# nullmax-vision/SimPB

Hardware: AMD Instinct MI355X
Metric: frames/sec (6-cam sample) + MSDeformAttn HBM GB/s, R50 704x256 @1/2/4/8 GPU (higher is better)
Workload: dtype f32

## Files before the change

### include/simpb_hip.h

```cpp
#ifndef SIMPB_HIP_H
#define SIMPB_HIP_H

#ifdef __cplusplus
extern "C" {
#endif

#define SIMPB_OK 0
#define SIMPB_EINVAL 1
#define SIMPB_ELAUNCH 2

#define SIMPB_RECORD3D_WIDTH 15

int simpb_abi_version(void);

const char* simpb_last_error(void);

#define SIMPB_KERNEL_DAF 1
#define SIMPB_KERNEL_MSDA 2
int simpb_timing_enable(int capacity);
int simpb_timing_read(int kernel_id, float* ms_out, int max_n);
void simpb_timing_reset(void);

int simpb_deformable_aggregation_forward(
    float* output, const float* mc_ms_feat, const int* spatial_shape, const int* scale_start_index,
// ... 77 lines not shown
                                       long long image_stride, int yoff, int iy, int irv, int igu, int igv, int ibu,
                                       void* stream);

int simpb_preprocess_mid_pitch(int out_width);

#define SIMPB_GEMM_MAX_SEGS 4
#define SIMPB_GEMM_MAX_JOBS 4
#define SIMPB_GEMM_OUT_F32 0
#define SIMPB_GEMM_OUT_SPLIT_HALFS 1
typedef struct simpb_gemm_job {
  const float* x[SIMPB_GEMM_MAX_SEGS];
  int ldx[SIMPB_GEMM_MAX_SEGS];
  int kseg[SIMPB_GEMM_MAX_SEGS];
  int num_seg;
  int M, N, K;
  const float* w;
  const float* bias;
  float* y;
  const int* m_live;
  int ldw, ldy, relu;
  int out_fmt;
  const int* row_flag;
  const float* bias2;
  const void* w_hi;
  const void* w_lo;
} simpb_gemm_job;
typedef struct simpb_gemm_args {
  int num_jobs;
  int reserved;
  simpb_gemm_job job[SIMPB_GEMM_MAX_JOBS];
} simpb_gemm_args;
int simpb_gemm_f32(const simpb_gemm_args* args, void* stream);

int simpb_layernorm_f32(float* out, int ldo, const float* x0, int ld0, int k0, const float* x1, int ld1, int k1,
                        const float* gamma, const float* beta, int num_rows, const int* m_live, void* stream);

#define SIMPB_MAX_LEVELS 8
int simpb_format_tokens(float* col_feats, const void* const* level_ptrs, const void* const* level_bias,
                        const int* level_hw, int num_levels, int num_images, int channels, int src_is_half, void* stream);

int simpb_bias_act_nhwc_f16(void* y, const void* bias, const void* residual, long long num_pixels, int channels,
                            int relu, void* stream);

int simpb_bias_relu_maxpool_nhwc_f16(void* y, const void* x, const void* bias, int num_images, int in_h, int in_w,
                                     int channels, void* stream);

int simpb_conv1x1_nhwc_f16(void* y, const void* x, const void* weight, const void* bias, const void* residual,
                           int num_images, int in_h, int in_w, int in_channels, int out_channels, int stride, int relu,
                           int residual_upsample2x, const void* input_bias, int variant, void* stream);

int simpb_conv3x3_nhwc_f16(void* y, float* tokens, void* tokens_f16, int tokens_per_cam, int level_start, const void* x,
                           const void* weight, const void* bias, int num_images, int in_h, int in_w, int in_channels,
                           int out_channels, int stride, int relu, int variant, void* stream);

int simpb_conv3x3_group_tokens_f16(int num_levels, float* tokens, void* tokens_f16, int tokens_per_cam, const int* level_start,
                                   const void* const* x, const void* const* weight, const void* const* bias, int num_images,
                                   const int* in_h, const int* in_w, int in_channels, int out_channels, int relu, void* stream);

int simpb_attention_f32(float* out, const float* q, const float* k, const float* v, const int* query_cam,
                        const int* group_start, int batch_size, int num_heads, int head_dim, int num_query,
                        int num_key, int ldq, int ldk, int ldv, int ldo, float scale, void* stream);

int simpb_attention_f32_split(float* out, const float* q, const float* k, const float* v, const int* query_cam,
                              const int* group_start, int batch_size, int num_heads, int head_dim, int num_query,
                              int num_key, int ldq, int ldk, int ldv, int ldo, float scale, void* stream);

int simpb_attention_split_halfs(float* out, const void* q, const void* k, const void* v, const int* query_cam,
                                const int* group_start, int batch_size, int num_heads, int head_dim, int num_query,
                                int num_key, int ldq, int ldk, int ldv, int ldo, void* stream);

#define SIMPB_MLP_MAX_OPS 12
#define SIMPB_MLP_MAX_CHAINS 8
#define SIMPB_MLP_POST_NONE 0
#define SIMPB_MLP_POST_REFINE3D 1
#define SIMPB_MLP_POST_REFINE2D 2
#define SIMPB_MLP_POST_SIGMOID 3
#define SIMPB_MLP_LINEAR 0
#define SIMPB_MLP_LAYERNORM 1
#define SIMPB_MLP_IN_ROWS 0
#define SIMPB_MLP_IN_SINE2D 1
#define SIMPB_MLP_IN_ROWS_LN 2
typedef struct simpb_mlp_op {
  int type, in_dim, out_dim, relu;
  const float* w;
  const float* b;
} simpb_mlp_op;
typedef struct simpb_mlp_chain {
  const float* x;
  const float* x2;
  float* out;
  const float* out_scale;
  int ldx, ldx2, ldo, in_dim, in_mode, n_ops;
  int post, ldres, res_cols, div_rows, div_col0, reserved;
  const float* res;
  const float* div;
  simpb_mlp_op ops[SIMPB_MLP_MAX_OPS];
  const float* ln_w;
  const float* ln_b;
  float* ln_out;
  int ld_ln_out, reserved2;
} simpb_mlp_chain;
typedef struct simpb_mlp_args {
  int num_rows, num_chains;
  int weights_transposed;
  int reserved;
  simpb_mlp_chain chain[SIMPB_MLP_MAX_CHAINS];
// ... 161 lines not shown
```

### simpb_amd/_lib.py

```python
import ctypes
import os

from .build import LIB

_lib = None

_P = ctypes.c_void_p
_I = ctypes.c_int
_F = ctypes.c_float
_LL = ctypes.c_longlong


class WorldTables(ctypes.Structure):
    _fields_ = [("class_range", _F * 32), ("attr_moving", ctypes.c_ubyte * 32), ("attr_still", ctypes.c_ubyte * 32),
                ("threshold", _F), ("has_threshold", _I), ("num_output", _I)]


SIGNATURES = {
    "simpb_abi_version": ([], _I),
    "simpb_last_error": ([], ctypes.c_char_p),
    "simpb_timing_enable": ([_I], _I),
    "simpb_timing_read": ([_I, _P, _I], _I),
    "simpb_timing_reset": ([], None),
    "simpb_deformable_aggregation_forward": ([_P] * 6 + [_I] * 8 + [_P], _I),
    "simpb_dfa_fused_forward": ([_P, _P, _I] + [_P] * 11 + [_I] * 9 + [_P], _I),
    "simpb_dfa_fused_forward_cams": ([_P, _P, _I] + [_P] * 11 + [_I] * 9 + [_P, _P], _I),
    "simpb_deformable_aggregation_backward": ([_P] * 9 + [_I] * 8 + [_P], _I),
    "simpb_ms_deform_attn_grouped_forward": ([_P] * 7 + [_I] * 8 + [_P], _I),
    "simpb_msda_linear_forward": ([_P, _I, _P, _I, _P, _P, _P, _I, _P, _I, _P, _P] + [_I] * 8 + [_P], _I),
    "simpb_ms_deform_attn_grouped_backward": ([_P] * 10 + [_I] * 8 + [_P], _I),
    "simpb_linear_f32": ([_P] * 4 + [_I] * 4 + [_P], _I),
    "simpb_linear_f16x3": ([_P] * 5 + [_I] * 3 + [_P], _I),
    "simpb_gemm_f32": ([_P, _P], _I),
    "simpb_layernorm_f32": ([_P, _I, _P, _I, _I, _P, _I, _I, _P, _P, _I, _P, _P], _I),
    "simpb_bias_act_nhwc_f16": ([_P, _P, _P, ctypes.c_longlong, _I, _I, _P], _I),
    "simpb_bias_relu_maxpool_nhwc_f16": ([_P, _P, _P, _I, _I, _I, _I, _P], _I),
    "simpb_conv1x1_nhwc_f16": ([_P] * 5 + [_I] * 8 + [_P, _I, _P], _I),
    "simpb_conv3x3_nhwc_f16": ([_P, _P, _P, _I, _I, _P, _P, _P] + [_I] * 8 + [_P], _I),
    "simpb_conv3x3_group_tokens_f16": ([_I, _P, _P, _I, _P, _P, _P, _P, _I, _P, _P, _I, _I, _I, _P], _I),
    "simpb_stem_conv7x7_pool_f16": ([_P] * 4 + [_I] * 4 + [_P], _I),
    "simpb_image_to_nhwc4_f16": ([_P, _P] + [ctypes.c_longlong] * 4 + [_I] * 4 + [_P], _I),
    "simpb_preprocess_u8_nhwc4_f16": ([_P] * 10 + [_I] * 11 + [_P], _I),
    "simpb_preprocess_yuv420sp_nhwc4_f16": ([_P] * 10 + [_I] * 18 + [_P], _I),
    "simpb_preprocess_surface_nhwc4_f16": ([_P] * 11 + [_I] * 12 + [_LL] * 4 + [_I] * 6 + [_P], _I),
    "simpb_preprocess_mid_pitch": ([_I], _I),
    "simpb_linear_f16in_split": ([_P] * 5 + [_I] * 3 + [_P], _I),
    "simpb_format_tokens": ([_P, _P, _P, _P, _I, _I, _I, _I, _P], _I),
    "simpb_attention_f32": ([_P] * 6 + [_I] * 9 + [_F, _P], _I),
    "simpb_attention_f32_split": ([_P] * 6 + [_I] * 9 + [_F, _P], _I),
    "simpb_attention_split_halfs": ([_P] * 6 + [_I] * 9 + [_P], _I),
    "simpb_mlp_chain_forward": ([_P, _P], _I),
    "simpb_bank_get": ([_P] * 6 + [_I] * 2 + [_F] * 2 + [_P], _I),
    "simpb_bank_update": ([_P] * 10 + [_I] * 5 + [_P], _I),
    "simpb_bank_update_rank": ([_P, _P] + [_I] * 4 + [_P], _I),
    "simpb_bank_update_merge": ([_P] * 13 + [_I, _P] + [_I] * 5 + [_P], _I),
    "simpb_bank_update_merge_active": ([_P] * 13 + [_I, _P] + [_I] * 5 + [_P, _P], _I),
    "simpb_bank_cache": ([_P] * 10 + [_I] * 6 + [_F, _I, _F, _P, _I, _P, _P], _I),
    "simpb_bank_cache_streams": ([_P] * 10 + [_I] * 6 + [_F, _I, _F, _P, _I, _P, _P, _P], _I),
    "simpb_bank_cache_streams_active": ([_P] * 10 + [_I] * 6 + [_F, _I, _F, _P, _I, _P, _P, _P, _P], _I),
    "simpb_decode3d_record": ([_P] * 6 + [_I] * 4 + [_P], _I),
    "simpb_decode2d_record": ([_P] * 6 + [_I] * 4 + [_F] * 4 + [_P], _I),
    "simpb_record2d_compact": ([_P, _LL, _P, _LL, _I, _I, _I, _P], _I),
    "simpb_decode2d_record_ragged": ([_P] * 7 + [_I] * 5 + [_F] * 4 + [_P], _I),
    "simpb_world_record": ([_P] * 5 + [WorldTables, _I, _P], _I),
    "simpb_topk_rows": ([_P, _P, _P, _I, _I, _I, _P], _I),
    "simpb_rowdot_sigmoid": ([_P, _P, _I, _P, _P, _I, _I, _P, _P], _I),
    "simpb_anchor_projection": ([_P] * 4 + [_I] * 2 + [_P], _I),
    "simpb_msda_prep": ([_P, _P, _P, _I, _P, _I, _P, _I, _I, _I, _I, _P, _P], _I),
    "simpb_dfa_points": ([_P] * 7 + [_I] * 5 + [_P], _I),
    "simpb_dfa_weights": ([_P] * 3 + [_I] * 6 + [_P], _I),
    "simpb_dfa_points_cams": ([_P] * 7 + [_I] * 5 + [_P, _P], _I),
    "simpb_dfa_weights_cams": ([_P] * 3 + [_I] * 6 + [_P, _P], _I),
    "simpb_alloc_project_cams": ([_P] * 5 + [_I] * 3 + [_F] * 5 + [_P, _P], _I),
    "simpb_alloc_project": ([_P] * 5 + [_I] * 3 + [_F] * 5 + [_P], _I),
    "simpb_alloc_compact": ([_P] * 3 + [_I] * 3 + [_P], _I),
    "simpb_alloc_group_start": ([_P] * 3 + [_I] * 3 + [_P], _I),
    "simpb_alloc_scatter": ([_P] * 12 + [_I] * 4 + [_F] * 2 + [_P], _I),
    "simpb_alloc_static": ([_P] * 15 + [_I] * 4 + [_F] * 5 + [_P], _I),
    "simpb_alloc_ragged": ([_P] * 15 + [_I] * 4 + [_F] * 5 + [_P], _I),
    "simpb_alloc_ragged_active": ([_P] * 15 + [_I] * 4 + [_F] * 5 + [_P, _P], _I),
    "simpb_alloc_static_cams": ([_P] * 15 + [_I] * 4 + [_F] * 5 + [_P, _P], _I),
    "simpb_alloc_ragged_cams": ([_P] * 15 + [_I] * 4 + [_F] * 5 + [_P, _P, _P], _I),
    "simpb_gather_rows": ([_P] * 3 + [_I] * 4 + [_P], _I),
    "simpb_aggregate_2d_to_3d": ([_P] * 8 + [_I] * 5 + [_P], _I),
    "simpb_aggregate_2d_to_3d_alpha": ([_P] * 9 + [_I, _I, _P, _P] + [_I] * 5 + [_P], _I),
}

ERRORS = {1: "SIMPB_EINVAL (bad pointer/size/layout)", 2: "SIMPB_ELAUNCH (kernel launch failed)"}


def lib():
# ... 23 lines not shown
```

### simpb_amd/csrc/conv1x1.hip

```cpp
#include <hip/hip_runtime.h>
#include <hip/hip_fp16.h>
#include <type_traits>
#include "../../include/simpb_hip.h"
#include "mfma_f16.h"

extern "C" int simpb_check_launch(void);
extern "C" int simpb_conv_pointwise_staged(void* y, const void* x, const void* weight, const void* bias, const void* residual,
                                           int p_out, int in_h, int in_w, int ho, int wo, int in_channels, int out_channels,
                                           int stride, int relu, int residual_upsample2x, int tiling, void* stream);

namespace {

using f32x16 = __attribute__((ext_vector_type(16))) float;
using h16x8 = __attribute__((ext_vector_type(8))) _Float16;

constexpr int BM = 128, BN = 64, BK = 64;
constexpr int LDH = BK + 8;
constexpr int LDC = BN + 1;
constexpr int kThreads = 256;

__device__ __forceinline__ int up2(int p, int Ho, int Wo) {
  const int n = p / (Ho * Wo), rem = p - n * (Ho * Wo);
  const int ho = rem / Wo, wo = rem - ho * Wo;
  return (n * (Ho >> 1) + (ho >> 1)) * (Wo >> 1) + (wo >> 1);
// ... 99 lines not shown
      __syncthreads();
      fetch(std::integral_constant<int, 1>{}, c + 3);
      multiply();
    }
  }

  __syncthreads();
#pragma unroll
  for (int n = 0; n < 2; ++n)
#pragma unroll
    for (int r = 0; r < 16; ++r) s_c[(wave * 32 + (r & 3) + 8 * (r >> 2) + 4 * kb) * LDC + n * 32 + r32] = acc[n][r];
  __syncthreads();
#pragma unroll
  for (int i = 0; i < 4; ++i) {
    const int idx = tid + i * kThreads;
    const int r = idx >> 3, c8 = (idx & 7) * 8;
    const int p = p0 + r;
    if (p >= P_out) continue;
    float v[8];
#pragma unroll
    for (int e = 0; e < 8; ++e) v[e] = s_c[r * LDC + c8 + e];
    if (full) {
      const h16x8 bv = *reinterpret_cast<const h16x8*>(bias + c0 + c8);
#pragma unroll
      for (int e = 0; e < 8; ++e) v[e] += (float)bv[e];
      if (residual) {
        const h16x8 rv = rres[i];
#pragma unroll
        for (int e = 0; e < 8; ++e) v[e] += (float)rv[e];
      }
      h16x8 o;
#pragma unroll
      for (int e = 0; e < 8; ++e) o[e] = (_Float16)(relu ? fmaxf(v[e], 0.f) : v[e]);
      *reinterpret_cast<h16x8*>(y + (size_t)p * Cout + c0 + c8) = o;
    } else {
#pragma unroll
      for (int e = 0; e < 8; ++e) {
        const int c = c0 + c8 + e;
        if (c < Cout) {
          float t = v[e] + (float)bias[c];
          if (residual) t += (float)residual[(size_t)(res_up ? up2(p, Ho, Wo) : p) * Cout + c];
          y[(size_t)p * Cout + c] = (_Float16)(relu ? fmaxf(t, 0.f) : t);
        }
      }
    }
  }
}

}

extern "C" int simpb_conv1x1_nhwc_f16(void* y, const void* x, const void* weight, const void* bias, const void* residual,
                                      int num_images, int in_h, int in_w, int in_channels, int out_channels, int stride,
                                      int relu, int residual_upsample2x, const void* input_bias, int variant, void* stream) {
  if (variant < 0 || variant > 3 || (input_bias && variant > 1)) return SIMPB_EINVAL;
  if (!y || !x || !weight || !bias || num_images <= 0 || in_h <= 0 || in_w <= 0 || in_channels <= 0 || out_channels <= 0 ||
      (stride != 1 && stride != 2) || in_channels % BK != 0 || out_channels % 8 != 0)
    return SIMPB_EINVAL;
  if ((reinterpret_cast<size_t>(y) | reinterpret_cast<size_t>(x) | reinterpret_cast<size_t>(weight) |
       reinterpret_cast<size_t>(bias) | reinterpret_cast<size_t>(residual) | reinterpret_cast<size_t>(input_bias)) & 15)
    return SIMPB_EINVAL;
  const int ho = (in_h - 1) / stride + 1, wo = (in_w - 1) / stride + 1;
  if (residual_upsample2x && (!residual || (ho & 1) || (wo & 1))) return SIMPB_EINVAL;
  const long long p_out = (long long)num_images * ho * wo;
  if (p_out > (1ll << 30)) return SIMPB_EINVAL;
  (void)hipGetLastError();
  if (variant == 0) {
    variant = (input_bias || in_channels < 512) ? 1 : 2;
  }
  if (variant > 1) {
    if ((long long)num_images * in_h * in_w * in_channels > (1ll << 31) - 1) return SIMPB_EINVAL;
    return simpb_conv_pointwise_staged(y, x, weight, bias, residual, (int)p_out, in_h, in_w, ho, wo, in_channels, out_channels,
                                       stride, relu, residual_upsample2x, variant - 2, stream);
  }
  dim3 grid((unsigned)((p_out + BM - 1) / BM), (out_channels + BN - 1) / BN);
  if (grid.y > 65535) return SIMPB_EINVAL;
  hipLaunchKernelGGL(conv1x1_f16_kernel, grid, dim3(kThreads), 0, static_cast<hipStream_t>(stream),
                     static_cast<_Float16*>(y), static_cast<const _Float16*>(x), static_cast<const _Float16*>(weight),
                     static_cast<const _Float16*>(bias), static_cast<const _Float16*>(residual), (int)p_out, in_channels,
                     out_channels, relu, stride, ho, wo, in_h, in_w, residual_upsample2x ? 1 : 0,
                     static_cast<const _Float16*>(input_bias));
  return simpb_check_launch();
}
```

### simpb_amd/csrc/conv3x3.hip

```cpp
#include <hip/hip_runtime.h>
#include <hip/hip_fp16.h>
#include <type_traits>
#include "../../include/simpb_hip.h"
#include "mfma_f16.h"

extern "C" int simpb_check_launch(void);

namespace {

using f32x16 = __attribute__((ext_vector_type(16))) float;
using h16x8 = __attribute__((ext_vector_type(8))) _Float16;

constexpr int BN = 64, BK = 64;
constexpr int LDH = BK + 8;
constexpr int LDC = BN + 1;
constexpr int kThreads = 256;
constexpr int kStageBytes = 2 * BN * LDH * 2;
constexpr int kTileBytes = 4 * 32 * LDC * 4;
constexpr int kSmemBytes = kStageBytes > kTileBytes ? kStageBytes : kTileBytes;

struct ConvArgs {
  _Float16* y;
  float* tok;
  _Float16* tok16;
// ... 243 lines not shown
    };
    for (int c = 0; c < nchunks; c += 3) {
      step(IC<0>{}, IC<1>{}, IC<2>{}, c);
      step(IC<1>{}, IC<2>{}, IC<0>{}, c + 1);
      step(IC<2>{}, IC<0>{}, IC<1>{}, c + 2);
    }
  }

  const bool full = c0 + BN <= a.Cout;
  auto emit = [&](int p, int c8, const float (&v)[8]) __attribute__((always_inline)) { emit_piece<TOK16>(a, c0, full, p, c8, v); };
  float* mine = s_c + wave * 32 * LDC;
#pragma unroll
  for (int f = 0; f < AF; ++f) {
    __syncthreads();
#pragma unroll
    for (int n = 0; n < 2; ++n)
#pragma unroll
      for (int r = 0; r < 16; ++r) mine[((r & 3) + 8 * (r >> 2) + 4 * kb) * LDC + n * 32 + r32] = acc[f][n][r];
    __syncthreads();
    if constexpr (KSPLIT) {
      const int r = tid >> 3, c8 = (tid & 7) * 8;
      float v[8];
#pragma unroll
      for (int e = 0; e < 8; ++e) {
        float s = 0.f;
#pragma unroll
        for (int w4 = 0; w4 < 4; ++w4) s += s_c[(w4 * 32 + r) * LDC + c8 + e];
        v[e] = s;
      }
      emit(p0 + 32 * f + r, c8, v);
    } else {
#pragma unroll
      for (int pass = 0; pass < 4; ++pass) {
        const int r = (lane >> 3) + 8 * pass, c8 = (lane & 7) * 8;
        float v[8];
#pragma unroll
        for (int e = 0; e < 8; ++e) v[e] = mine[r * LDC + c8 + e];
        emit(p0 + row0 + 32 * f + r, c8, v);
      }
    }
  }
}

template <int AF, bool KSPLIT, bool TOK16>
void launch(ConvArgs& a, hipStream_t stream) {
  constexpr int BMt = KSPLIT ? 32 * AF : 128 * AF;
  a.gx = (a.P_out + BMt - 1) / BMt;
  a.gy = (a.Cout + BN - 1) / BN;
  const long long total = (long long)a.gx * a.gy;
  a.per_xcd = (int)((total + 7) / 8);
  hipLaunchKernelGGL((conv3x3_f16_kernel<AF, KSPLIT, TOK16>), dim3((unsigned)(a.per_xcd * 8)), dim3(kThreads), 0, stream, a);
}


template <int BMt, int BNt, int WGM, int WGN, int TAPS, bool TOK16>
__device__ __forceinline__ void conv_staged_tile(const ConvArgs& a, const int tile) {
  constexpr int NT = 64 * WGM * WGN;
  constexpr int AF = BMt / WGM / 32, NF = BNt / WGN / 32;
  static_assert(AF * WGM * 32 == BMt && NF * WGN * 32 == BNt && NF <= 2, "tile = waves x 32-row / 32-column fragments");
  constexpr int NA = (BMt * 8 + NT - 1) / NT, NB = (BNt * 8 + NT - 1) / NT;
  constexpr int kRows = BMt + BNt;
  constexpr int LDW = 32 * NF + 1;
  constexpr int kStage = 2 * kRows * LDH * 2, kTile = WGM * WGN * 32 * LDW * 4;
  __shared__ __attribute__((aligned(16))) unsigned char smem[kStage > kTile ? kStage : kTile];
  _Float16* s_ab = reinterpret_cast<_Float16*>(smem);
  float* s_c = reinterpret_cast<float*>(smem);

  const int tx = tile / a.gy, ty = tile - tx * a.gy;
  const int tid = threadIdx.x;
  const int lane = tid & 63, wave = tid >> 6;
  const int r32 = lane & 31, kb = lane >> 5;
  const int wm = wave / WGN, wn = wave - wm * WGN;
  const int p0 = tx * BMt, c0 = ty * BNt;
  const int Cin = a.Cin, W = a.W, H = a.H;
  const int per_tap = Cin / BK, nchunks = TAPS * per_tap;
  const size_t K = (size_t)TAPS * Cin;
  const _Float16* __restrict__ wgt = a.w;

  const int sc = (tid & 7) * 8;
  const _Float16* actr[NA];
  unsigned amask = 0;
  static_assert(NA <= 5, "6 mask bits per staged row in one register");
#pragma unroll
  for (int i = 0; i < NA; ++i) {
    const int p = min(p0 + ((tid + NT * i) >> 3), a.P_out - 1);
    const int hw = a.Ho * a.Wo;
    const int n = p / hw, rem = p - n * hw;
    const int ho = rem / a.Wo, wo = rem - ho * a.Wo;
    const int hc = ho * a.stride, wc = wo * a.stride;
    actr[i] = a.x + ((size_t)(n * H + hc) * W + wc) * Cin + sc;
    const unsigned rows = (hc > 0 ? 1u : 0u) | 2u | (hc + 1 < H ? 4u : 0u), cols = (wc > 0 ? 1u : 0u) | 2u | (wc + 1 < W ? 4u : 0u);
    amask |= (rows | (cols << 3)) << (6 * i);
  }
  size_t brow[NB];
#pragma unroll
  for (int i = 0; i < NB; ++i) brow[i] = (size_t)min(c0 + ((tid + NT * i) >> 3), a.Cout - 1) * K + sc;

  h16x8 ra[3][NA], rb[3][NB];
  unsigned alive[3];

  auto fetch = [&](auto set_c, int chunk) __attribute__((always_inline)) {
    constexpr int s = decltype(set_c)::value;
    const int c = min(chunk, nchunks - 1);
    if constexpr (TAPS == 1) {
      const int k0 = c * BK;
#pragma unroll
      for (int i = 0; i < NA; ++i) ra[s][i] = *reinterpret_cast<const h16x8*>(actr[i] + k0);
      alive[s] = ~0u;
#pragma unroll
      for (int i = 0; i < NB; ++i) rb[s][i] = *reinterpret_cast<const h16x8*>(wgt + brow[i] + k0);
    } else {
      const int tap = c / per_tap, k0 = (c - tap * per_tap) * BK;
      const int dy = tap / 3, dx = tap - dy * 3;
      const int toff = ((dy - 1) * W + (dx - 1)) * Cin;
      unsigned m = 0;
#pragma unroll
      for (int i = 0; i < NA; ++i) {
        const bool in = ((amask >> (6 * i + dy)) & (amask >> (6 * i + 3 + dx)) & 1u) != 0;
        m |= (in ? 1u : 0u) << i;
        ra[s][i] = *reinterpret_cast<const h16x8*>(actr[i] + (in ? toff : 0) + k0);
      }
      alive[s] = m;
      const size_t koff = (size_t)tap * Cin + k0;
#pragma unroll
      for (int i = 0; i < NB; ++i) rb[s][i] = *reinterpret_cast<const h16x8*>(wgt + brow[i] + koff);
    }
  };
  auto stash = [&](auto set_c, int buf) __attribute__((always_inline)) {
    constexpr int s = decltype(set_c)::value;
    const h16x8 zero = {0, 0, 0, 0, 0, 0, 0, 0};
    _Float16* base = s_ab + buf * kRows * LDH;
#pragma unroll
    for (int i = 0; i < NA; ++i) {
      const int idx = tid + NT * i;
      if ((BMt * 8) % NT == 0 || idx < BMt * 8)
        *reinterpret_cast<h16x8*>(&base[(idx >> 3) * LDH + sc]) = ((alive[s] >> i) & 1u) ? ra[s][i] : zero;
    }
#pragma unroll
    for (int i = 0; i < NB; ++i) {
      const int idx = tid + NT * i;
      if ((BNt * 8) % NT == 0 || idx < BNt * 8) *reinterpret_cast<h16x8*>(&base[(BMt + (idx >> 3)) * LDH + sc]) = rb[s][i];
    }
  };

  f32x16 acc[AF][NF];
#pragma unroll
  for (int f = 0; f < AF; ++f)
#pragma unroll
    for (int n = 0; n < NF; ++n)
#pragma unroll
      for (int r = 0; r < 16; ++r) acc[f][n][r] = 0.f;

  auto multiply = [&](int buf) __attribute__((always_inline)) {
    const _Float16* sa = s_ab + buf * kRows * LDH + (wm * AF * 32 + r32) * LDH + 8 * kb;
    const _Float16* sb = s_ab + buf * kRows * LDH + (BMt + wn * NF * 32 + r32) * LDH + 8 * kb;
#pragma unroll
    for (int ks = 0; ks < BK / 16; ++ks) {
      h16x8 av[AF], bv[NF];
#pragma unroll
      for (int f = 0; f < AF; ++f) av[f] = *reinterpret_cast<const h16x8*>(sa + f * 32 * LDH + 16 * ks);
#pragma unroll
      for (int n = 0; n < NF; ++n) bv[n] = *reinterpret_cast<const h16x8*>(sb + n * 32 * LDH + 16 * ks);
#pragma unroll
      for (int f = 0; f < AF; ++f)
#pragma unroll
        for (int n = 0; n < NF; ++n) acc[f][n] = simpb::mfma_32x32x16_f16(av[f], bv[n], acc[f][n]);
    }
  };

  fetch(IC<0>{}, 0);
  fetch(IC<1>{}, 1);
  fetch(IC<2>{}, 2);
  __builtin_amdgcn_sched_barrier(0);
  stash(IC<0>{}, 0);
  __syncthreads();
  auto step = [&](auto cur, auto nxt, int c) __attribute__((always_inline)) {
    fetch(cur, c + 3);
    __builtin_amdgcn_sched_barrier(0);
    stash(nxt, (c + 1) & 1);
    __builtin_amdgcn_sched_barrier(0);
    multiply(c & 1);
    __syncthreads();
  };
  for (int c = 0; c < nchunks; c += 3) {
    step(IC<0>{}, IC<1>{}, c);
    if (TAPS == 9 || c + 1 < nchunks) step(IC<1>{}, IC<2>{}, c + 1);
    if (TAPS == 9 || c + 2 < nchunks) step(IC<2>{}, IC<0>{}, c + 2);
  }

  float* mine = s_c + wave * 32 * LDW;
  const int cw = c0 + wn * NF * 32;
  const bool full = cw + 32 * NF <= a.Cout;
#pragma unroll
  for (int f = 0; f < AF; ++f) {
    if (f) __syncthreads();
#pragma unroll
    for (int n = 0; n < NF; ++n)
#pragma unroll
      for (int r = 0; r < 16; ++r) mine[((r & 3) + 8 * (r >> 2) + 4 * kb) * LDW + n * 32 + r32] = acc[f][n][r];
    __syncthreads();
    constexpr int PR = 4 * NF;
#pragma unroll
    for (int pass = 0; pass < 32 * PR / 64; ++pass) {
      const int idx = lane + 64 * pass;
      const int r = idx / PR, c8 = (idx % PR) * 8;
      float v[8];
#pragma unroll
      for (int e = 0; e < 8; ++e) v[e] = mine[r * LDW + c8 + e];
      emit_piece<TOK16>(a, cw, full, p0 + (wm * AF + f) * 32 + r, c8, v);
    }
  }
}

template <int BMt, int BNt, int WGM, int WGN, int TAPS, bool TOK16>
__global__ __launch_bounds__(64 * WGM * WGN, WGM * WGN == 3 ? 3 : 2) void conv_staged_kernel(const ConvArgs a) {
  const int tile = (blockIdx.x & 7) * a.per_xcd + (blockIdx.x >> 3);
  if ((int)(blockIdx.x >> 3) >= a.per_xcd || tile >= a.gx * a.gy) return;
  conv_staged_tile<BMt, BNt, WGM, WGN, TAPS, TOK16>(a, tile);
}

constexpr int kMaxConvGroup = 4;
struct ConvGroup {
  ConvArgs a[kMaxConvGroup];
  int start[kMaxConvGroup + 1];
  int n, per_xcd;
};
template <int BMt, int BNt, int WGM, int WGN, int TAPS, bool TOK16>
__global__ __launch_bounds__(64 * WGM * WGN, WGM * WGN == 3 ? 3 : 2) void conv_staged_group_kernel(const ConvGroup g) {
  const int gt = (blockIdx.x & 7) * g.per_xcd + (blockIdx.x >> 3);
  if ((int)(blockIdx.x >> 3) >= g.per_xcd || gt >= g.start[g.n]) return;
  int j = 0;
#pragma unroll
  for (int t = 1; t < kMaxConvGroup; ++t)
    if (t < g.n && gt >= g.start[t]) j = t;
  conv_staged_tile<BMt, BNt, WGM, WGN, TAPS, TOK16>(g.a[j], gt - g.start[j]);
}

template <int BMt, int BNt, int WGM, int WGN, int TAPS, bool TOK16>
void launch_staged(ConvArgs& a, hipStream_t stream) {
  a.gx = (a.P_out + BMt - 1) / BMt;
  a.gy = (a.Cout + BNt - 1) / BNt;
  const long long total = (long long)a.gx * a.gy;
  a.per_xcd = (int)((total + 7) / 8);
  hipLaunchKernelGGL((conv_staged_kernel<BMt, BNt, WGM, WGN, TAPS, TOK16>), dim3((unsigned)(a.per_xcd * 8)), dim3(64 * WGM * WGN), 0,
                     stream, a);
}

}

extern "C" int simpb_conv3x3_nhwc_f16(void* y, float* tokens, void* tokens_f16, int tokens_per_cam, int level_start,
                                      const void* x, const void* weight, const void* bias, int num_images, int in_h, int in_w,
                                      int in_channels, int out_channels, int stride, int relu, int variant, void* stream) {
  const bool to_tokens = tokens || tokens_f16;
  if ((!y && !to_tokens) || (y && to_tokens) || (reinterpret_cast<size_t>(tokens_f16) & 15) || !x || !weight || !bias || num_images <= 0 || in_h <= 0 || in_w <= 0 ||
      in_channels <= 0 || out_channels <= 0 || (stride != 1 && stride != 2) || in_channels % BK != 0 || out_channels % 8 != 0 ||
      variant < 0 || variant > 8)
    return SIMPB_EINVAL;
  if ((reinterpret_cast<size_t>(y) | reinterpret_cast<size_t>(tokens) | reinterpret_cast<size_t>(x) |
       reinterpret_cast<size_t>(weight) | reinterpret_cast<size_t>(bias)) & 15)
    return SIMPB_EINVAL;
  const int ho = (in_h - 1) / stride + 1, wo = (in_w - 1) / stride + 1;
  const long long p_out = (long long)num_images * ho * wo;
  const long long in_elems = (long long)num_images * in_h * in_w * in_channels;
  if (p_out > (1ll << 30) || in_elems > (1ll << 31) - 1) return SIMPB_EINVAL;
  if (to_tokens && (tokens_per_cam < ho * wo || level_start < 0 || level_start + ho * wo > tokens_per_cam)) return SIMPB_EINVAL;
  (void)hipGetLastError();
  ConvArgs a{static_cast<_Float16*>(y), tokens, static_cast<_Float16*>(tokens_f16), static_cast<const _Float16*>(x), static_cast<const _Float16*>(weight),
             static_cast<const _Float16*>(bias), nullptr, 0, (int)p_out, in_channels, out_channels, relu, stride, ho, wo, in_h, in_w,
             tokens_per_cam, level_start, 0, 0, 0};
  const long long ny = (out_channels + BN - 1) / BN;
  if (variant == 0) {
    const long long t96 = (p_out + 95) / 96, t128 = (p_out + 127) / 128, t64 = (p_out + 63) / 64;
    if (out_channels >= 128 && t128 * ((out_channels + 127) / 128) >= 2048) variant = 6;
    else if (out_channels >= 128 && t96 * ((out_channels + 127) / 128) >= 160) variant = 8;
    else if (t96 * ny >= 256) variant = 7;
    else if (t128 * ny >= 128) variant = 1;
    else if (t64 * ny >= 128) variant = 4;
    else variant = 3;
  }
  hipStream_t s = static_cast<hipStream_t>(stream);
  auto dispatch = [&](auto tok16_c) {
    constexpr bool T = decltype(tok16_c)::value;
    switch (variant) {
      case 1: launch<1, false, T>(a, s); break;
      case 2: launch<2, false, T>(a, s); break;
      case 3: launch<1, true, T>(a, s); break;
      case 4: launch<2, true, T>(a, s); break;
      case 5: launch_staged<128, 64, 4, 1, 9, T>(a, s); break;
      case 6: launch_staged<128, 128, 2, 2, 9, T>(a, s); break;
      case 7: launch_staged<96, 64, 3, 1, 9, T>(a, s); break;
      default: launch_staged<96, 128, 1, 4, 9, T>(a, s); break;
    }
  };
  if (!tokens && tokens_f16) dispatch(std::true_type{});
  else dispatch(std::false_type{});
  return simpb_check_launch();
}

extern "C" int simpb_conv3x3_group_tokens_f16(int num_levels, float* tokens, void* tokens_f16, int tokens_per_cam,
                                              const int* level_start, const void* const* x, const void* const* weight,
                                              const void* const* bias, int num_images, const int* in_h, const int* in_w,
                                              int in_channels, int out_channels, int relu, void* stream) {
  if (num_levels < 1 || num_levels > kMaxConvGroup || (!tokens && !tokens_f16) || !level_start || !x || !weight || !bias || !in_h || !in_w ||
      num_images <= 0 || in_channels <= 0 || out_channels <= 0 || in_channels % BK != 0 || out_channels % 8 != 0 ||
      ((reinterpret_cast<size_t>(tokens) | reinterpret_cast<size_t>(tokens_f16)) & 15))
    return SIMPB_EINVAL;
  ConvGroup g{};
  long long total = 0;
  for (int j = 0; j < num_levels; ++j) {
    if (!x[j] || !weight[j] || !bias[j] || in_h[j] <= 0 || in_w[j] <= 0 ||
        ((reinterpret_cast<size_t>(x[j]) | reinterpret_cast<size_t>(weight[j]) | reinterpret_cast<size_t>(bias[j])) & 15))
      return SIMPB_EINVAL;
    const long long p_out = (long long)num_images * in_h[j] * in_w[j];
    if (p_out > (1ll << 30) || p_out * in_channels > (1ll << 31) - 1) return SIMPB_EINVAL;
    if (tokens_per_cam < in_h[j] * in_w[j] || level_start[j] < 0 || level_start[j] + in_h[j] * in_w[j] > tokens_per_cam)
      return SIMPB_EINVAL;
    g.a[j] = ConvArgs{nullptr, tokens, static_cast<_Float16*>(tokens_f16), static_cast<const _Float16*>(x[j]),
                      static_cast<const _Float16*>(weight[j]), static_cast<const _Float16*>(bias[j]), nullptr, 0, (int)p_out,
                      in_channels, out_channels, relu, 1, in_h[j], in_w[j], in_h[j], in_w[j], tokens_per_cam, level_start[j],
                      0, 0, 0};
    g.a[j].gx = (int)((p_out + 95) / 96);
    g.a[j].gy = (out_channels + 127) / 128;
    g.start[j] = (int)total;
    total += (long long)g.a[j].gx * g.a[j].gy;
  }
  if (total > (1 << 24)) return SIMPB_EINVAL;
  for (int j = num_levels; j <= kMaxConvGroup; ++j) g.start[j] = (int)total;
  g.n = num_levels;
  g.per_xcd = (int)((total + 7) / 8);
  (void)hipGetLastError();
  if (!tokens)
    hipLaunchKernelGGL((conv_staged_group_kernel<96, 128, 1, 4, 9, true>), dim3((unsigned)(g.per_xcd * 8)), dim3(256), 0,
                       static_cast<hipStream_t>(stream), g);
  else
    hipLaunchKernelGGL((conv_staged_group_kernel<96, 128, 1, 4, 9, false>), dim3((unsigned)(g.per_xcd * 8)), dim3(256), 0,
                       static_cast<hipStream_t>(stream), g);
  return simpb_check_launch();
}

extern "C" int simpb_conv_pointwise_staged(void* y, const void* x, const void* weight, const void* bias, const void* residual,
                                           int p_out, int in_h, int in_w, int ho, int wo, int in_channels, int out_channels,
                                           int stride, int relu, int residual_upsample2x, int tiling, void* stream) {
  ConvArgs a{static_cast<_Float16*>(y), nullptr, nullptr, static_cast<const _Float16*>(x), static_cast<const _Float16*>(weight),
             static_cast<const _Float16*>(bias), static_cast<const _Float16*>(residual), residual_upsample2x ? 1 : 0,
             p_out, in_channels, out_channels, relu, stride, ho, wo, in_h, in_w, 0, 0, 0, 0, 0};
  hipStream_t s = static_cast<hipStream_t>(stream);
  if (tiling == 0) launch_staged<128, 64, 4, 1, 1, false>(a, s);
  else launch_staged<128, 128, 2, 2, 1, false>(a, s);
  return simpb_check_launch();
}
```

### simpb_amd/plugin/ops.py

```python
import ctypes

import torch
from torch.autograd.function import Function

from .. import _lib


def _ptr(t):
    return ctypes.c_void_p(t.data_ptr())


def _stream():
    return ctypes.c_void_p(torch.cuda.current_stream().cuda_stream)


def _require_gpu(*tensors):
    for t in tensors:
        if not t.is_cuda:
            raise RuntimeError("simpb_amd operators run on the GPU only (got a CPU tensor); "
                               "there is no CPU fallback")


_layout_ok = {}

# ... 395 lines not shown
    if residual_upsample2x and (residual is None or ho % 2 or wo % 2):
        raise ValueError("residual_upsample2x needs a residual and even output sizes")
    if residual is not None and (tuple(residual.shape) != tuple(want) or residual.dtype != torch.float16
                                 or not residual.is_contiguous(memory_format=torch.channels_last)):
        raise ValueError("residual must match the output (channels_last f16)")
    if input_bias is not None and (input_bias.dtype != torch.float16 or input_bias.numel() != cin or not input_bias.is_contiguous()):
        raise ValueError("input_bias must be a contiguous f16 [Cin] tensor")
    w2 = weight.reshape(cout, cin)
    if not w2.is_contiguous():
        w2 = w2.contiguous()
    status = _lib.lib().simpb_conv1x1_nhwc_f16(_ptr(y), _ptr(x), _ptr(w2), _ptr(bias), _ptr(residual) if residual is not None else None,
                                               n, h, w, cin, cout, stride, 1 if relu else 0,
                                               1 if residual_upsample2x else 0,
                                               _ptr(input_bias) if input_bias is not None else None, variant, _stream())
    _lib.check(status, "simpb_conv1x1_nhwc_f16")
    return y


def conv3x3_nhwc(x, weight, bias, relu=True, stride=1, tokens=None, variant=0):
    _require_gpu(x, weight, bias)
    n, cin, h, w = x.shape
    cout = weight.shape[0]
    if (x.dtype != torch.float16 or not x.is_contiguous(memory_format=torch.channels_last) or weight.dtype != torch.float16
            or bias.dtype != torch.float16 or tuple(weight.shape) != (cout, cin, 3, 3) or cin % 64 or cout % 8
            or stride not in (1, 2) or bias.numel() != cout or not bias.is_contiguous()):
        raise ValueError("conv3x3_nhwc takes channels_last f16 input, f16 [Cout, Cin, 3, 3] weight, Cin % 64 == 0, Cout % 8 == 0")
    if not weight.is_contiguous(memory_format=torch.channels_last):
        weight = weight.contiguous(memory_format=torch.channels_last)
    ho, wo = (h - 1) // stride + 1, (w - 1) // stride + 1
    col16 = None
    if tokens is None:
        y = torch.empty((n, cout, ho, wo), device=x.device, dtype=torch.float16, memory_format=torch.channels_last)
        col, per_cam, start = None, 0, 0
    else:
        col, per_cam, start = tokens[:3]
        col16 = tokens[3] if len(tokens) > 3 else None
        y = None
        if col is None and col16 is None:
            raise ValueError("tokens: an f32 or an f16 token buffer")
        if col16 is not None and (col16.dtype != torch.float16 or not col16.is_contiguous()
                                  or (col is not None and col16.shape != col.shape)):
            raise ValueError("tokens: the f16 buffer must match col_feats")
        rows = col if col is not None else col16
        if ((col is not None and col.dtype != torch.float32) or not rows.is_contiguous() or rows.shape[-1] != cout
                or rows.numel() != n * per_cam * cout or start < 0 or start + ho * wo > per_cam):
            raise ValueError("tokens: (contiguous f32 [bs, cams * tokens_per_cam, Cout] with bs * cams == N, tokens_per_cam, level_start)")
    status = _lib.lib().simpb_conv3x3_nhwc_f16(_ptr(y) if y is not None else None, _ptr(col) if col is not None else None,
                                               _ptr(col16) if col16 is not None else None, per_cam, start, _ptr(x), _ptr(weight), _ptr(bias), n, h, w, cin, cout, stride,
                                               1 if relu else 0, variant, _stream())
    _lib.check(status, "simpb_conv3x3_nhwc_f16")
    return y


def conv3x3_group_tokens(xs, weights, biases, col, per_cam, starts, col16=None, relu=False):
    import ctypes
    if col is None and col16 is None:
        raise ValueError("conv3x3_group_tokens: an f32 or an f16 token buffer")
    rows = col if col is not None else col16
    _require_gpu(*xs, *weights, *biases, rows)
    n, cin = xs[0].shape[:2]
    cout = weights[0].shape[0]
    k = len(xs)
    if not (1 <= k <= 4 and len(weights) == k and len(biases) == k and len(starts) == k):
        raise ValueError("conv3x3_group_tokens: 1..4 levels, one weight / bias / start each")
    ws = []
    for x, w, b in zip(xs, weights, biases):
        if (x.dtype != torch.float16 or not x.is_contiguous(memory_format=torch.channels_last) or x.shape[0] != n or x.shape[1] != cin
                or w.dtype != torch.float16 or tuple(w.shape) != (cout, cin, 3, 3) or b.dtype != torch.float16 or b.numel() != cout
                or not b.is_contiguous() or cin % 64 or cout % 8):
            raise ValueError("conv3x3_group_tokens takes channels_last f16 inputs of one channel count, f16 [Cout, Cin, 3, 3] weights")
        ws.append(w if w.is_contiguous(memory_format=torch.channels_last) else w.contiguous(memory_format=torch.channels_last))
    if ((col is not None and col.dtype != torch.float32) or not rows.is_contiguous() or rows.shape[-1] != cout
            or rows.numel() != n * per_cam * cout
            or (col16 is not None and (col16.dtype != torch.float16 or not col16.is_contiguous() or col16.shape != rows.shape))):
        raise ValueError("conv3x3_group_tokens: col = contiguous f32 [bs, cams * tokens_per_cam, Cout] with bs * cams == N")
    arr_p, arr_i = ctypes.c_void_p * k, ctypes.c_int * k
    status = _lib.lib().simpb_conv3x3_group_tokens_f16(
        k, _ptr(col) if col is not None else None, _ptr(col16) if col16 is not None else None, int(per_cam), arr_i(*[int(v) for v in starts]),
        arr_p(*[x.data_ptr() for x in xs]), arr_p(*[w.data_ptr() for w in ws]), arr_p(*[b.data_ptr() for b in biases]), n,
        arr_i(*[x.shape[2] for x in xs]), arr_i(*[x.shape[3] for x in xs]), cin, cout, 1 if relu else 0, _stream())
    _lib.check(status, "simpb_conv3x3_group_tokens_f16")


def _stem_weight_packed(weight):
    tag = (weight.data_ptr(), weight._version, str(weight.device))
    hit = getattr(weight, "_simpb_stem_pack", None)
    if hit is None or hit[0] != tag:
        with torch.no_grad():
            w = weight.detach().float()
            full = torch.zeros(64, 4, 7, 8, device=w.device)
            full[:, :3, :, :7] = w
            pack = full.reshape(64, 4, 7, 4, 2).permute(2, 3, 4, 0, 1).contiguous().half()
        hit = (tag, pack)
        weight._simpb_stem_pack = hit
    return hit[1]


def stem_conv_pool(img, weight, bias):
    _require_gpu(img, weight, bias)
    n, c, h, w = img.shape
    if img.dtype != torch.float32 or c != 3 or tuple(weight.shape) != (64, 3, 7, 7) or bias.numel() != 64 or h < 1 or w < 1:
        raise ValueError("stem_conv_pool: f32 [N, 3, H, W] image, [64, 3, 7, 7] weight, 64 biases")
    lib = _lib.lib()
    x4 = torch.empty(n, h, w, 4, device=img.device, dtype=torch.float16)
    _lib.check(lib.simpb_image_to_nhwc4_f16(_ptr(x4), _ptr(img), img.stride(0), img.stride(1), img.stride(2), img.stride(3), n, c, h, w,
                                            _stream()), "simpb_image_to_nhwc4_f16")
# ... 75 lines not shown
```

Baseline: 411.9.

## Add split-K staged conv3x3 kernels and small-tile 1x1 path for deep layers

Adds a K-split variant of the staged conv kernel in which several thread groups in one block each take an interleaved share of the K chunks, stage them in separate shared-memory slices, and sum their partial tiles before the epilogue. It adds new 64x64 tile variants for conv3x3 (9-11) and a 64x64 tiling for the 1x1 path (variant 4). It also moves the conv3x3 heuristic into an exported chooser that now picks these variants for wide, low-tile-count layers. The aim is to fill the GPU on deep ResNet stages where few output tiles exist, at the cost of a cross-group reduction and a larger shared-memory footprint.

```diff
diff --git a/include/simpb_hip.h b/include/simpb_hip.h
--- a/include/simpb_hip.h
+++ b/include/simpb_hip.h
@@ -153,6 +153,8 @@
 int simpb_conv3x3_nhwc_f16(void* y, float* tokens, void* tokens_f16, int tokens_per_cam, int level_start, const void* x,
                            const void* weight, const void* bias, int num_images, int in_h, int in_w, int in_channels,
                            int out_channels, int stride, int relu, int variant, void* stream);
+
+int simpb_conv3x3_choose_variant(long long p_out, int in_channels, int out_channels);
 
 int simpb_conv3x3_group_tokens_f16(int num_levels, float* tokens, void* tokens_f16, int tokens_per_cam, const int* level_start,
                                    const void* const* x, const void* const* weight, const void* const* bias, int num_images,
diff --git a/simpb_amd/_lib.py b/simpb_amd/_lib.py
--- a/simpb_amd/_lib.py
+++ b/simpb_amd/_lib.py
@@ -37,6 +37,7 @@
     "simpb_bias_relu_maxpool_nhwc_f16": ([_P, _P, _P, _I, _I, _I, _I, _P], _I),
     "simpb_conv1x1_nhwc_f16": ([_P] * 5 + [_I] * 8 + [_P, _I, _P], _I),
     "simpb_conv3x3_nhwc_f16": ([_P, _P, _P, _I, _I, _P, _P, _P] + [_I] * 8 + [_P], _I),
+    "simpb_conv3x3_choose_variant": ([_LL, _I, _I], _I),
     "simpb_conv3x3_group_tokens_f16": ([_I, _P, _P, _I, _P, _P, _P, _P, _I, _P, _P, _I, _I, _I, _P], _I),
     "simpb_stem_conv7x7_pool_f16": ([_P] * 4 + [_I] * 4 + [_P], _I),
     "simpb_image_to_nhwc4_f16": ([_P, _P] + [ctypes.c_longlong] * 4 + [_I] * 4 + [_P], _I),
diff --git a/simpb_amd/csrc/conv1x1.hip b/simpb_amd/csrc/conv1x1.hip
--- a/simpb_amd/csrc/conv1x1.hip
+++ b/simpb_amd/csrc/conv1x1.hip
@@ -175,7 +175,7 @@
 extern "C" int simpb_conv1x1_nhwc_f16(void* y, const void* x, const void* weight, const void* bias, const void* residual,
                                       int num_images, int in_h, int in_w, int in_channels, int out_channels, int stride,
                                       int relu, int residual_upsample2x, const void* input_bias, int variant, void* stream) {
-  if (variant < 0 || variant > 3 || (input_bias && variant > 1)) return SIMPB_EINVAL;
+  if (variant < 0 || variant > 4 || (input_bias && variant > 1)) return SIMPB_EINVAL;
   if (!y || !x || !weight || !bias || num_images <= 0 || in_h <= 0 || in_w <= 0 || in_channels <= 0 || out_channels <= 0 ||
       (stride != 1 && stride != 2) || in_channels % BK != 0 || out_channels % 8 != 0)
     return SIMPB_EINVAL;
@@ -189,6 +189,10 @@
   (void)hipGetLastError();
   if (variant == 0) {
     variant = (input_bias || in_channels < 512) ? 1 : 2;
+    if (variant == 2 && in_channels >= 1024) {
+      const long long t128 = ((p_out + 127) / 128) * ((out_channels + 63) / 64);
+      if (t128 < 320) variant = 4;
+    }
   }
   if (variant > 1) {
     if ((long long)num_images * in_h * in_w * in_channels > (1ll << 31) - 1) return SIMPB_EINVAL;
diff --git a/simpb_amd/csrc/conv3x3.hip b/simpb_amd/csrc/conv3x3.hip
--- a/simpb_amd/csrc/conv3x3.hip
+++ b/simpb_amd/csrc/conv3x3.hip
@@ -319,8 +319,7 @@
   hipLaunchKernelGGL((conv3x3_f16_kernel<AF, KSPLIT, TOK16>), dim3((unsigned)(a.per_xcd * 8)), dim3(kThreads), 0, stream, a);
 }
 
-
-template <int BMt, int BNt, int WGM, int WGN, int TAPS, bool TOK16>
+template <int BMt, int BNt, int WGM, int WGN, int TAPS, bool TOK16, int KS = 1, bool DIRECTK = false>
 __device__ __forceinline__ void conv_staged_tile(const ConvArgs& a, const int tile) {
   constexpr int NT = 64 * WGM * WGN;
   constexpr int AF = BMt / WGM / 32, NF = BNt / WGN / 32;
@@ -328,19 +327,21 @@
   constexpr int NA = (BMt * 8 + NT - 1) / NT, NB = (BNt * 8 + NT - 1) / NT;
   constexpr int kRows = BMt + BNt;
   constexpr int LDW = 32 * NF + 1;
-  constexpr int kStage = 2 * kRows * LDH * 2, kTile = WGM * WGN * 32 * LDW * 4;
+  constexpr int kStage = KS * 2 * kRows * LDH * 2, kTile = KS * WGM * WGN * 32 * LDW * 4;
   __shared__ __attribute__((aligned(16))) unsigned char smem[kStage > kTile ? kStage : kTile];
-  _Float16* s_ab = reinterpret_cast<_Float16*>(smem);
+  const int grp = KS > 1 ? (int)threadIdx.x / NT : 0;
+  _Float16* s_ab = reinterpret_cast<_Float16*>(smem) + grp * (2 * kRows * LDH);
   float* s_c = reinterpret_cast<float*>(smem);
 
   const int tx = tile / a.gy, ty = tile - tx * a.gy;
-  const int tid = threadIdx.x;
+  const int tid = threadIdx.x - grp * NT;
   const int lane = tid & 63, wave = tid >> 6;
   const int r32 = lane & 31, kb = lane >> 5;
   const int wm = wave / WGN, wn = wave - wm * WGN;
   const int p0 = tx * BMt, c0 = ty * BNt;
   const int Cin = a.Cin, W = a.W, H = a.H;
   const int per_tap = Cin / BK, nchunks = TAPS * per_tap;
+  const int nsteps = (nchunks + KS - 1) / KS;
   const size_t K = (size_t)TAPS * Cin;
   const _Float16* __restrict__ wgt = a.w;
 
@@ -366,14 +367,16 @@
   h16x8 ra[3][NA], rb[3][NB];
   unsigned alive[3];
 
-  auto fetch = [&](auto set_c, int chunk) __attribute__((always_inline)) {
+  auto fetch = [&](auto set_c, int step_i) __attribute__((always_inline)) {
     constexpr int s = decltype(set_c)::value;
+    const int chunk = step_i * KS + grp;
+    const bool exists = KS == 1 || chunk < nchunks;
     const int c = min(chunk, nchunks - 1);
     if constexpr (TAPS == 1) {
       const int k0 = c * BK;
 #pragma unroll
       for (int i = 0; i < NA; ++i) ra[s][i] = *reinterpret_cast<const h16x8*>(actr[i] + k0);
-      alive[s] = ~0u;
+      alive[s] = exists ? ~0u : 0u;
 #pragma unroll
       for (int i = 0; i < NB; ++i) rb[s][i] = *reinterpret_cast<const h16x8*>(wgt + brow[i] + k0);
     } else {
@@ -387,7 +390,7 @@
         m |= (in ? 1u : 0u) << i;
         ra[s][i] = *reinterpret_cast<const h16x8*>(actr[i] + (in ? toff : 0) + k0);
       }
-      alive[s] = m;
+      alive[s] = exists ? m : 0u;
       const size_t koff = (size_t)tap * Cin + k0;
 #pragma unroll
       for (int i = 0; i < NB; ++i) rb[s][i] = *reinterpret_cast<const h16x8*>(wgt + brow[i] + koff);
@@ -419,15 +422,16 @@
       for (int r = 0; r < 16; ++r) acc[f][n][r] = 0.f;
 
   auto multiply = [&](int buf) __attribute__((always_inline)) {
-    const _Float16* sa = s_ab + buf * kRows * LDH + (wm * AF * 32 + r32) * LDH + 8 * kb;
-    const _Float16* sb = s_ab + buf * kRows * LDH + (BMt + wn * NF * 32 + r32) * LDH + 8 * kb;
+    constexpr int KLANE = DIRECTK ? 32 : 8, KSTEP = DIRECTK ? 8 : 16;
+    const _Float16* sa = s_ab + buf * kRows * LDH + (wm * AF * 32 + r32) * LDH + KLANE * kb;
+    const _Float16* sb = s_ab + buf * kRows * LDH + (BMt + wn * NF * 32 + r32) * LDH + KLANE * kb;
 #pragma unroll
     for (int ks = 0; ks < BK / 16; ++ks) {
       h16x8 av[AF], bv[NF];
 #pragma unroll
-      for (int f = 0; f < AF; ++f) av[f] = *reinterpret_cast<const h16x8*>(sa + f * 32 * LDH + 16 * ks);
-#pragma unroll
-      for (int n = 0; n < NF; ++n) bv[n] = *reinterpret_cast<const h16x8*>(sb + n * 32 * LDH + 16 * ks);
+      for (int f = 0; f < AF; ++f) av[f] = *reinterpret_cast<const h16x8*>(sa + f * 32 * LDH + KSTEP * ks);
+#pragma unroll
+      for (int n = 0; n < NF; ++n) bv[n] = *reinterpret_cast<const h16x8*>(sb + n * 32 * LDH + KSTEP * ks);
 #pragma unroll
       for (int f = 0; f < AF; ++f)
 #pragma unroll
@@ -449,13 +453,13 @@
     multiply(c & 1);
     __syncthreads();
   };
-  for (int c = 0; c < nchunks; c += 3) {
+  for (int c = 0; c < nsteps; c += 3) {
     step(IC<0>{}, IC<1>{}, c);
-    if (TAPS == 9 || c + 1 < nchunks) step(IC<1>{}, IC<2>{}, c + 1);
-    if (TAPS == 9 || c + 2 < nchunks) step(IC<2>{}, IC<0>{}, c + 2);
-  }
-
-  float* mine = s_c + wave * 32 * LDW;
+    if ((TAPS == 9 && KS == 1) || c + 1 < nsteps) step(IC<1>{}, IC<2>{}, c + 1);
+    if ((TAPS == 9 && KS == 1) || c + 2 < nsteps) step(IC<2>{}, IC<0>{}, c + 2);
+  }
+
+  float* mine = s_c + (grp * WGM * WGN + wave) * 32 * LDW;
   const int cw = c0 + wn * NF * 32;
   const bool full = cw + 32 * NF <= a.Cout;
 #pragma unroll
@@ -467,6 +471,7 @@
       for (int r = 0; r < 16; ++r) mine[((r & 3) + 8 * (r >> 2) + 4 * kb) * LDW + n * 32 + r32] = acc[f][n][r];
     __syncthreads();
     constexpr int PR = 4 * NF;
+    if (KS > 1 && grp) continue;
 #pragma unroll
     for (int pass = 0; pass < 32 * PR / 64; ++pass) {
       const int idx = lane + 64 * pass;
@@ -474,6 +479,12 @@
       float v[8];
 #pragma unroll
       for (int e = 0; e < 8; ++e) v[e] = mine[r * LDW + c8 + e];
+      if constexpr (KS > 1) {
+#pragma unroll
+        for (int g = 1; g < KS; ++g)
+#pragma unroll
+          for (int e = 0; e < 8; ++e) v[e] += mine[(g * WGM * WGN * 32 + r) * LDW + c8 + e];
+      }
       emit_piece<TOK16>(a, cw, full, p0 + (wm * AF + f) * 32 + r, c8, v);
     }
   }
@@ -484,6 +495,13 @@
   const int tile = (blockIdx.x & 7) * a.per_xcd + (blockIdx.x >> 3);
   if ((int)(blockIdx.x >> 3) >= a.per_xcd || tile >= a.gx * a.gy) return;
   conv_staged_tile<BMt, BNt, WGM, WGN, TAPS, TOK16>(a, tile);
+}
+
+template <int BMt, int BNt, int WGM, int WGN, int TAPS, bool TOK16, int KS>
+__global__ __launch_bounds__(64 * WGM * WGN * KS, 2) void conv_staged_ksplit_kernel(const ConvArgs a) {
+  const int tile = (blockIdx.x & 7) * a.per_xcd + (blockIdx.x >> 3);
+  if ((int)(blockIdx.x >> 3) >= a.per_xcd || tile >= a.gx * a.gy) return;
+  conv_staged_tile<BMt, BNt, WGM, WGN, TAPS, TOK16, KS, true>(a, tile);
 }
 
 constexpr int kMaxConvGroup = 4;
@@ -513,6 +531,27 @@
                      stream, a);
 }
 
+template <int BMt, int BNt, int WGM, int WGN, int TAPS, bool TOK16, int KS>
+void launch_staged_ksplit(ConvArgs& a, hipStream_t stream) {
+  a.gx = (a.P_out + BMt - 1) / BMt;
+  a.gy = (a.Cout + BNt - 1) / BNt;
+  const long long total = (long long)a.gx * a.gy;
+  a.per_xcd = (int)((total + 7) / 8);
+  hipLaunchKernelGGL((conv_staged_ksplit_kernel<BMt, BNt, WGM, WGN, TAPS, TOK16, KS>), dim3((unsigned)(a.per_xcd * 8)),
+                     dim3(64 * WGM * WGN * KS), 0, stream, a);
+}
+
+}
+
+extern "C" int simpb_conv3x3_choose_variant(long long p_out, int in_channels, int out_channels) {
+  const long long ny = (out_channels + BN - 1) / BN;
+  const long long t96 = (p_out + 95) / 96, t128 = (p_out + 127) / 128, t64 = (p_out + 63) / 64;
+  if (out_channels >= 128 && t128 * ((out_channels + 127) / 128) >= 2048) return 6;
+  if (out_channels >= 128 && t96 * ((out_channels + 127) / 128) >= 160) return 8;
+  if (t96 * ny >= 256) return 7;
+  if (t128 * ny >= 128) return in_channels >= 256 && out_channels >= 256 ? 9 : 1;
+  if (t64 * ny >= 128) return in_channels >= 512 && out_channels >= 512 ? 11 : 4;
+  return 3;
 }
 
 extern "C" int simpb_conv3x3_nhwc_f16(void* y, float* tokens, void* tokens_f16, int tokens_per_cam, int level_start,
@@ -521,7 +560,7 @@
   const bool to_tokens = tokens || tokens_f16;
   if ((!y && !to_tokens) || (y && to_tokens) || (reinterpret_cast<size_t>(tokens_f16) & 15) || !x || !weight || !bias || num_images <= 0 || in_h <= 0 || in_w <= 0 ||
       in_channels <= 0 || out_channels <= 0 || (stride != 1 && stride != 2) || in_channels % BK != 0 || out_channels % 8 != 0 ||
-      variant < 0 || variant > 8)
+      variant < 0 || variant > 11)
     return SIMPB_EINVAL;
   if ((reinterpret_cast<size_t>(y) | reinterpret_cast<size_t>(tokens) | reinterpret_cast<size_t>(x) |
        reinterpret_cast<size_t>(weight) | reinterpret_cast<size_t>(bias)) & 15)
@@ -535,16 +574,7 @@
   ConvArgs a{static_cast<_Float16*>(y), tokens, static_cast<_Float16*>(tokens_f16), static_cast<const _Float16*>(x), static_cast<const _Float16*>(weight),
              static_cast<const _Float16*>(bias), nullptr, 0, (int)p_out, in_channels, out_channels, relu, stride, ho, wo, in_h, in_w,
              tokens_per_cam, level_start, 0, 0, 0};
-  const long long ny = (out_channels + BN - 1) / BN;
-  if (variant == 0) {
-    const long long t96 = (p_out + 95) / 96, t128 = (p_out + 127) / 128, t64 = (p_out + 63) / 64;
-    if (out_channels >= 128 && t128 * ((out_channels + 127) / 128) >= 2048) variant = 6;
-    else if (out_channels >= 128 && t96 * ((out_channels + 127) / 128) >= 160) variant = 8;
-    else if (t96 * ny >= 256) variant = 7;
-    else if (t128 * ny >= 128) variant = 1;
-    else if (t64 * ny >= 128) variant = 4;
-    else variant = 3;
-  }
+  if (variant == 0) variant = simpb_conv3x3_choose_variant(p_out, in_channels, out_channels);
   hipStream_t s = static_cast<hipStream_t>(stream);
   auto dispatch = [&](auto tok16_c) {
     constexpr bool T = decltype(tok16_c)::value;
@@ -556,7 +586,10 @@
       case 5: launch_staged<128, 64, 4, 1, 9, T>(a, s); break;
       case 6: launch_staged<128, 128, 2, 2, 9, T>(a, s); break;
       case 7: launch_staged<96, 64, 3, 1, 9, T>(a, s); break;
-      default: launch_staged<96, 128, 1, 4, 9, T>(a, s); break;
+      case 8: launch_staged<96, 128, 1, 4, 9, T>(a, s); break;
+      case 9: launch_staged_ksplit<64, 64, 2, 2, 9, T, 1>(a, s); break;
+      case 10: launch_staged_ksplit<64, 64, 2, 2, 9, T, 2>(a, s); break;
+      default: launch_staged_ksplit<64, 64, 2, 2, 9, T, 4>(a, s); break;
     }
   };
   if (!tokens && tokens_f16) dispatch(std::true_type{});
@@ -613,6 +646,7 @@
              p_out, in_channels, out_channels, relu, stride, ho, wo, in_h, in_w, 0, 0, 0, 0, 0};
   hipStream_t s = static_cast<hipStream_t>(stream);
   if (tiling == 0) launch_staged<128, 64, 4, 1, 1, false>(a, s);
-  else launch_staged<128, 128, 2, 2, 1, false>(a, s);
+  else if (tiling == 1) launch_staged<128, 128, 2, 2, 1, false>(a, s);
+  else launch_staged<64, 64, 2, 2, 1, false>(a, s);
   return simpb_check_launch();
 }
diff --git a/simpb_amd/plugin/ops.py b/simpb_amd/plugin/ops.py
--- a/simpb_amd/plugin/ops.py
+++ b/simpb_amd/plugin/ops.py
@@ -471,6 +471,10 @@
     return y
 
 
+def conv3x3_variant_for(p_out, in_channels, out_channels):
+    return int(_lib.lib().simpb_conv3x3_choose_variant(int(p_out), int(in_channels), int(out_channels)))
+
+
 def conv3x3_group_tokens(xs, weights, biases, col, per_cam, starts, col16=None, relu=False):
     import ctypes
     if col is None and col16 is None:
```

New measurement: 433.2, median of 6. 1.05x the previous value.
